# old-dab/rtlsdr

Hardware: NVIDIA B200
Metric: input Msamples/s (higher is better)
Workload: dtype int16/int64 fixed point

## Files before the change

### rtlsdr_b200/csrc/scan_abi.cu

```cuda
#include "../../include/rtlsdr_gpu_scan.h"
#include "csv_text.cuh"
#include "scan_kernels.cuh"
#include "scan_large.cuh"

#include <algorithm>
#include <cmath>
#include <cstdio>
#include <cstdlib>
#include <cstring>
#include <new>
#include <string>
#include <vector>

using namespace rscan;

namespace {

constexpr int kDescSlots = 4;
constexpr size_t kDefaultRing = 32u << 20;
constexpr size_t kScratchBudget = 512ull << 20;
constexpr int kChainMaxPasses = 7;
constexpr int kChainCap0 = 8192;
constexpr int kDecimChunks = 4;
constexpr size_t kDecimOverlapBytes = 1ull << 30;

enum Path { PATH_RMS, PATH_SMALL_U8, PATH_SMALL_DECIM, PATH_LARGE };

struct DescSlot {
	void *h = nullptr;
	void *d = nullptr;
	size_t cap = 0;
	cudaEvent_t done = nullptr;
	bool used = false;
};

struct RegularKey {
	const void *base = nullptr;
	int hop_first = -1, hop_count = 0, passes = 0;
	long long pass_stride = 0, hop_stride = 0;
	bool valid = false;
	int n_reads = 0, n_segs = 0;
	bool operator==(const RegularKey &o) const
	{
		return valid && o.valid && base == o.base && hop_first == o.hop_first && hop_count == o.hop_count &&
		       passes == o.passes && pass_stride == o.pass_stride && hop_stride == o.hop_stride;
	}
};

}

struct rtlsdr_gpu_scan {
	rtlsdr_gpu_scan_cfg_t cfg;
	int N = 1;
	Path path = PATH_SMALL_U8;
	int l_len = 0, n_blocks = 0, blocks_padded = 0, samples_per_read = 0;
	long long image_stride = 0;
	int db_i1 = 0, db_i2 = 0, db_count = 2;
	int num_sms = 148, ctas_per_sm = 2;

	cudaStream_t own_stream = nullptr, stream = nullptr;
	cudaEvent_t ev_a = nullptr, ev_b = nullptr;

	long long *d_avg = nullptr;
	long long *d_smp64 = nullptr;
	long long *d_avg_other = nullptr;
	cudaStream_t report_stream = nullptr;
	cudaEvent_t ev_scan = nullptr, ev_report[2] = { nullptr, nullptr };
	bool report_pending[2] = { false, false };
	int cur_acc = 0;
	unsigned *d_done = nullptr;
	unsigned long long *d_level = nullptr;
	std::vector<uint64_t> level_bytes;
	int2 *d_tw = nullptr;
	int2 *d_twc = nullptr;
	int2 *d_twb = nullptr;
	uint16_t *d_win = nullptr;
	double *d_db = nullptr;
	double *d_iir = nullptr;
	int *d_samples = nullptr;
	int *h_samples_pinned = nullptr;
	std::vector<int> samples;
	PassTw tw0;
	std::vector<int2> tw_host;

	size_t ring_bytes = 0;
	int ring_reads = 0;
	uint8_t *h_ring[2] = { nullptr, nullptr };
	uint8_t *d_ring[2] = { nullptr, nullptr };
	cudaEvent_t ring_done[2] = { nullptr, nullptr };
	bool ring_busy[2] = { false, false };
	int cur_half = 0;
	std::vector<int> ring_hops;
	std::vector<uint8_t> hop_shadow;

	DescSlot desc[kDescSlots];
	int desc_next = 0;
	struct RegCache {
		RegularKey key;
		void *d_desc = nullptr;
		size_t cap = 0;
		std::vector<int4> segs;
		uint64_t stamp = 0;
	};
	std::vector<RegCache> reg_cache;
	uint64_t reg_stamp = 0;
	cudaStream_t aux[2] = { nullptr, nullptr };
	cudaEvent_t fork_ev = nullptr, join_ev[2] = { nullptr, nullptr };
	cudaStream_t hb_head_stream = nullptr;
	cudaEvent_t hb_fork = nullptr, hb_join = nullptr;
	cudaStream_t copy_stream = nullptr;
	cudaEvent_t bulk_free = nullptr;
	bool bulk_used = false;
	std::vector<cudaEvent_t> chunk_ready;

	uint8_t *d_scratch = nullptr;
	size_t scratch_bytes = 0;

	uint8_t *d_bulk = nullptr;
	size_t bulk_bytes = 0;

	int2 *d_csv_cols = nullptr;
	int csv_rows = 0;
	double csv_step = 0.0;
	char *d_csv_slots = nullptr;
	size_t csv_slot_bytes = 0;
	int *d_csv_lens = nullptr;
	char *d_csv_text = nullptr;
	size_t csv_text_bytes = 0;
	long long *d_csv_len = nullptr;
	long long *h_csv_len = nullptr;

	bool last_was_epilogue = false;
	bool samples_on_device = false;
	uint64_t launches = 0, h2d = 0, d2h = 0;
	std::vector<std::pair<cudaEvent_t, cudaEvent_t>> timed;
	std::vector<cudaEvent_t> ev_pool;
	bool timing = false;
	int timing_every = 1;
	uint64_t timing_count = 0;

	int dbg_boxcar_mode = -1;
	int dbg_stagger_ns = 0;
	bool dbg_no_fused_boxcar = false, dbg_no_hb_stream = false, dbg_rms_warp = false;
	int dbg_large_pipe = 1;

	std::string last_error;
};

namespace {

#define CU(call)                                                                                 \
	do {                                                                                         \
		cudaError_t _e = (call);                                                                 \
		if (_e != cudaSuccess) {                                                                 \
			h->last_error = std::string(#call) + ": " + cudaGetErrorString(_e);                  \
			return RTLSDR_GPU_ERR_CUDA;                                                          \
		}                                                                                        \
	} while (0)

// ... 172 lines not shown
		return 0;
	}
	std::vector<int> count(tc + 1, 0);
	for (int i = 0; i < n; i++)
		count[hops[i] + 1]++;
	for (int i = 0; i < tc; i++)
		count[i + 1] += count[i];
	s_offs.resize(n);
	s_hops.resize(n);
	std::vector<int> cursor(count.begin(), count.end() - 1);
	for (int i = 0; i < n; i++) {
		int p = cursor[hops[i]]++;
		s_offs[p] = offs[i];
		s_hops[p] = hops[i];
	}
	segs.clear();
	if (h->path == PATH_SMALL_U8 || h->path == PATH_RMS || h->path == PATH_LARGE)
		return 0;
	const bool big_decim = h->path == PATH_SMALL_DECIM && (size_t)n * (size_t)h->cfg.buf_len >= kDecimOverlapBytes;
	const int target = std::max(1, h->num_sms * h->ctas_per_sm) * (big_decim ? kDecimChunks : 1);
	int chunk = std::max(1, (n + target - 1) / target);
	{
		const double per_seg = 0.35;
		double best = 1e300;
		int best_chunk = chunk;
		for (int k = 1; k <= 16; k++) {
			const int c = std::max(1, (chunk + k - 1) / k);
			long long nseg = 0;
			for (int hp = 0; hp < tc; hp++) {
				const int cnt = count[hp + 1] - count[hp];
				nseg += (cnt + c - 1) / c;
			}
			const long long rounds = (nseg + target - 1) / target;
			const double cost = (double)rounds * (c + per_seg);
			if (cost < best * 0.98) {
				best = cost;
				best_chunk = c;
			}
			if (c == 1)
				break;
		}
		chunk = best_chunk;
	}
	for (int hp = 0; hp < tc; hp++) {
		int lo = count[hp], hi = count[hp + 1];
		int cnt = hi - lo;
		if (cnt <= 0)
			continue;
		int pieces = (cnt + chunk - 1) / chunk;
		for (int k = 0; k < pieces; k++) {
			int a = lo + (int)((long long)cnt * k / pieces), b = lo + (int)((long long)cnt * (k + 1) / pieces);
			if (b > a)
				segs.push_back(make_int4(hp, a, b - a, 0));
		}
	}
	return (int)segs.size();
}


int large_process(rtlsdr_gpu_scan *h, const uint8_t *base, const long long *d_offs, const int *d_hops, int n_reads);

template <class K, class P>
int launch_after_epilogue(rtlsdr_gpu_scan *h, K kern, int grid, int block, int smem, const P &prm, bool allow_pdl = true)
{
	if (allow_pdl && h->last_was_epilogue && h->stream == h->own_stream) {
		cudaLaunchConfig_t cfg = {};
		cfg.gridDim = dim3(grid);
		cfg.blockDim = dim3(block);
		cfg.dynamicSmemBytes = smem;
		cfg.stream = h->stream;
		cudaLaunchAttribute attr[1];
		attr[0].id = cudaLaunchAttributeProgrammaticStreamSerialization;
		attr[0].val.programmaticStreamSerializationAllowed = 1;
		cfg.attrs = attr;
		cfg.numAttrs = 1;
		CU(cudaLaunchKernelEx(&cfg, kern, prm));
	} else {
		kern<<<grid, block, smem, h->stream>>>(prm);
	}
	h->last_was_epilogue = false;
	return 0;
}

template <int L, bool PEAK, bool IN16>
int launch_small_t(rtlsdr_gpu_scan *h, const SmallParams &prm)
{
	auto kern = scan_small_kernel<L, PEAK, IN16>;
	const int smem = SmallSmem<L>::bytes;
	static bool attr_set[64] = { false };
	if (h->cfg.device >= 64 || !attr_set[h->cfg.device]) {
		CU(cudaFuncSetAttribute(kern, cudaFuncAttributeMaxDynamicSharedMemorySize, smem));
		if (h->cfg.device < 64)
			attr_set[h->cfg.device] = true;
	}
	const int grid = IN16 ? std::min(prm.n_segs, h->num_sms * 8)
			      : (int)std::min<long long>(2ll * prm.n_entries, (long long)h->num_sms * h->ctas_per_sm);
	if (int rc = launch_after_epilogue(h, kern, grid, kThreads, smem, prm, !IN16))
		return rc;
	return check_launch(h, "scan_small_kernel");
}

template <int L>
int launch_small_l(rtlsdr_gpu_scan *h, const SmallParams &prm, bool in16)
{
	if (h->cfg.peak_hold)
		return in16 ? launch_small_t<L, true, true>(h, prm) : launch_small_t<L, true, false>(h, prm);
	return in16 ? launch_small_t<L, false, true>(h, prm) : launch_small_t<L, false, false>(h, prm);
}

int launch_small(rtlsdr_gpu_scan *h, const SmallParams &prm, bool in16)
{
	switch (h->cfg.bin_e) {
	case 1: return launch_small_l<1>(h, prm, in16);
	case 2: return launch_small_l<2>(h, prm, in16);
	case 3: return launch_small_l<3>(h, prm, in16);
	case 4: return launch_small_l<4>(h, prm, in16);
	case 5: return launch_small_l<5>(h, prm, in16);
	case 6: return launch_small_l<6>(h, prm, in16);
	case 7: return launch_small_l<7>(h, prm, in16);
	case 8: return launch_small_l<8>(h, prm, in16);
	case 9: return launch_small_l<9>(h, prm, in16);
	case 10: return launch_small_l<10>(h, prm, in16);
	case 11: return launch_small_l<11>(h, prm, in16);
	case 12: return launch_small_l<12>(h, prm, in16);
	default: break;
	}
	return RTLSDR_GPU_ERR_CONFIG;
}

template <int L, bool PEAK, int NS>
int launch_fused_boxcar_t(rtlsdr_gpu_scan *h, const FusedBoxcarParams &prm)
{
	auto k = scan_boxcar_fused_kernel<L, PEAK, NS>;
	const int smem = FusedSmem<L>::bytes(prm.ds, NS);
	const int grid = std::min(prm.n_segs, h->num_sms * 8);
	CU(cudaFuncSetAttribute(k, cudaFuncAttributeMaxDynamicSharedMemorySize, smem));
	if (int rc = launch_after_epilogue(h, k, grid, kThreads, smem, prm))
		return rc;
	return check_launch(h, "scan_boxcar_fused_kernel");
}

template <int L>
int launch_fused_boxcar_l(rtlsdr_gpu_scan *h, const FusedBoxcarParams &prm_in)
{
	FusedBoxcarParams prm = prm_in;
	const int limit = 227 * 1024 - 1024;
	int slots;
	if (2 * (FusedSmem<L>::bytes(prm.ds, 4) + 1024) <= 227 * 1024) {
		slots = 4;
	} else if (2 * (FusedSmem<L>::bytes(prm.ds, 3) + 1024) <= 227 * 1024) {
		slots = 3;
	} else {
		const int fit = (limit - FusedSmem<L>::off_stage) / (512 * prm.ds);
		slots = fit >= 12 ? 12 : fit >= 8 ? 8 : fit >= 6 ? 6 : fit >= 4 ? 4 : fit >= 3 ? 3 : 2;
	}
	prm.slots = slots;
	const bool pk = h->cfg.peak_hold != 0;
#define FUSED_CASE(NSV)                                                                               \
	case NSV:                                                                                     \
		return pk ? launch_fused_boxcar_t<L, true, NSV>(h, prm) : launch_fused_boxcar_t<L, false, NSV>(h, prm)
	switch (slots) {
		FUSED_CASE(12);
		FUSED_CASE(8);
		FUSED_CASE(6);
		FUSED_CASE(4);
		FUSED_CASE(3);
	default:
		return pk ? launch_fused_boxcar_t<L, true, 2>(h, prm) : launch_fused_boxcar_t<L, false, 2>(h, prm);
	}
#undef FUSED_CASE
}

constexpr int kStreamMinDs = 2;
constexpr int kStreamOneFftGroupDs = 24;

template <int L, int FG>
int stream_boxcar_slots(int ds)
{
	const int fit = (227 * 1024 - StreamSmem<L, FG>::off_stage) / (512 * ds);
	return std::min(fit, kStreamMaxSlots);
}

template <int L, bool PEAK, int FG, int BG>
int launch_stream_boxcar_t(rtlsdr_gpu_scan *h, const FusedBoxcarParams &prm_in)
{
	FusedBoxcarParams prm = prm_in;
	prm.slots = stream_boxcar_slots<L, FG>(prm.ds);
// ... 884 lines not shown
		delete h;
		return RTLSDR_GPU_ERR_CONFIG;
	}
	h->db_count = h->db_i2 - h->db_i1 + 2;

	int rc = RTLSDR_GPU_ERR_CUDA;
	do {
		if (cudaStreamCreateWithFlags(&h->own_stream, cudaStreamNonBlocking) != cudaSuccess)
			break;
		h->stream = h->own_stream;
		const size_t avg_bytes = ((size_t)cfg->tune_count * N + (size_t)cfg->tune_count) * sizeof(long long);
		if (cudaMalloc(&h->d_avg, avg_bytes) != cudaSuccess ||
		    cudaMalloc(&h->d_db, (size_t)cfg->tune_count * h->db_count * sizeof(double)) != cudaSuccess ||
		    cudaMalloc(&h->d_samples, (size_t)cfg->tune_count * sizeof(int)) != cudaSuccess ||
		    cudaMallocHost(&h->h_samples_pinned, (size_t)cfg->tune_count * sizeof(int)) != cudaSuccess) {
			rc = RTLSDR_GPU_ERR_NOMEM;
			break;
		}
		h->d_smp64 = h->d_avg + (size_t)cfg->tune_count * N;
		if (cfg->flags & RTLSDR_GPU_FLAG_ASYNC_REPORT) {
			if (cudaMalloc(&h->d_avg_other, avg_bytes) != cudaSuccess) {
				rc = RTLSDR_GPU_ERR_NOMEM;
				break;
			}
			if (cudaMemsetAsync(h->d_avg_other, 0, avg_bytes, h->stream) != cudaSuccess ||
			    cudaStreamCreateWithFlags(&h->report_stream, cudaStreamNonBlocking) != cudaSuccess ||
			    cudaEventCreateWithFlags(&h->ev_scan, cudaEventDisableTiming) != cudaSuccess ||
			    cudaEventCreateWithFlags(&h->ev_report[0], cudaEventDisableTiming) != cudaSuccess ||
			    cudaEventCreateWithFlags(&h->ev_report[1], cudaEventDisableTiming) != cudaSuccess)
				break;
		}
		if (cudaMalloc(&h->d_done, (size_t)cfg->tune_count * sizeof(unsigned)) != cudaSuccess) {
			rc = RTLSDR_GPU_ERR_NOMEM;
			break;
		}
		if (cudaMemsetAsync(h->d_done, 0, (size_t)cfg->tune_count * sizeof(unsigned), h->stream) != cudaSuccess)
			break;
		if (cudaMemsetAsync(h->d_avg, 0, avg_bytes, h->stream) != cudaSuccess)
			break;
		if (cfg->iir_alpha > 0.0) {
			const size_t ib = (size_t)cfg->tune_count * (size_t)(h->db_count - 1) * sizeof(double);
			if (cudaMalloc(&h->d_iir, ib) != cudaSuccess) {
				rc = RTLSDR_GPU_ERR_NOMEM;
				break;
			}
			if (cudaMemsetAsync(h->d_iir, 0xFF, ib, h->stream) != cudaSuccess)
				break;
		}
		if (cfg->flags & RTLSDR_GPU_FLAG_LEVEL_STATS) {
			const size_t lb = (size_t)cfg->tune_count * 2 * sizeof(unsigned long long);
			if (cudaMalloc(&h->d_level, lb) != cudaSuccess) {
				rc = RTLSDR_GPU_ERR_NOMEM;
				break;
			}
			if (cudaMemsetAsync(h->d_level, 0, lb, h->stream) != cudaSuccess)
				break;
			h->level_bytes.assign(cfg->tune_count, 0);
		}

		if (cfg->bin_e > 0) {
			std::vector<int16_t> sine((size_t)N * 3 / 4 + 4, 0);
			if (cfg->sinewave)
				memcpy(sine.data(), cfg->sinewave, ((size_t)N * 3 / 4) * sizeof(int16_t));
			else
				host_sine_table(cfg->bin_e, sine.data());
			const int half = std::max(N / 2, 1);
			h->tw_host.resize(half);
			for (int j = 0; j < half; j++) {
				int16_t wr = (int16_t)(sine[j + N / 4] >> 1);
				int16_t wi = (int16_t)((int16_t)(-sine[j]) >> 1);
				h->tw_host[j] = make_int2(wr, wi);
			}
			if (h->tw_host[0].y != 0 || (N >= 4 && h->tw_host[N / 4].x != 0)) {
				rc = RTLSDR_GPU_ERR_CONFIG;
				break;
			}
			memset(&h->tw0, 0, sizeof(h->tw0));
			for (int b = 0; b < 4 && b < cfg->bin_e; b++)
				for (int g = 0; g < (1 << b); g++)
					h->tw0.w[(1 << b) - 1 + g] = h->tw_host[(size_t)g << (cfg->bin_e - 1 - b)];
			std::vector<uint16_t> win(N);
			for (int i = 0; i < N; i++)
				win[i] = (uint16_t)((cfg->window_coefs ? cfg->window_coefs[i] : 256) & 0xFFFF);
			if (cudaMalloc(&h->d_tw, (size_t)half * sizeof(int2)) != cudaSuccess ||
			    cudaMalloc(&h->d_win, (size_t)N * sizeof(uint16_t)) != cudaSuccess) {
				rc = RTLSDR_GPU_ERR_NOMEM;
				break;
			}
			if (cudaMemcpy(h->d_tw, h->tw_host.data(), (size_t)half * sizeof(int2), cudaMemcpyHostToDevice) != cudaSuccess ||
			    cudaMemcpy(h->d_win, win.data(), (size_t)N * sizeof(uint16_t), cudaMemcpyHostToDevice) != cudaSuccess)
				break;
		}

		if (cfg->bin_e > 4 && cfg->bin_e <= 12) {
			const int L = cfg->bin_e;
			std::vector<int2> twc((size_t)N - 16);
			for (int st = 4; st < L; st++)
				for (int m = 0; m < (1 << st); m++)
					twc[(size_t)(1 << st) - 16 + m] = h->tw_host[(size_t)m << (L - 1 - st)];
			if (cudaMalloc(&h->d_twc, twc.size() * sizeof(int2)) != cudaSuccess) {
				rc = RTLSDR_GPU_ERR_NOMEM;
				break;
			}
			if (cudaMemcpy(h->d_twc, twc.data(), twc.size() * sizeof(int2), cudaMemcpyHostToDevice) != cudaSuccess)
				break;
		}
		if (h->path == PATH_LARGE) {
			std::vector<int2> twc(240);
			for (int st = 4; st < 8; st++)
				for (int m = 0; m < (1 << st); m++)
					twc[(size_t)(1 << st) - 16 + m] = h->tw_host[(size_t)m << (cfg->bin_e - 1 - st)];
			if (cudaMalloc(&h->d_twc, twc.size() * sizeof(int2)) != cudaSuccess) {
				rc = RTLSDR_GPU_ERR_NOMEM;
				break;
			}
			if (cudaMemcpy(h->d_twc, twc.data(), twc.size() * sizeof(int2), cudaMemcpyHostToDevice) != cudaSuccess)
				break;
		}
		if (h->path == PATH_LARGE) {
			const int L = cfg->bin_e, lb = std::min(8, L - 8);
			std::vector<int2> twb((size_t)256 * 240, make_int2(0, 0));
			for (int se = 4; se < lb; se++)
				for (int plow = 0; plow < 256; plow++)
					for (int ilow = 0; ilow < (1 << se); ilow++)
						twb[(size_t)256 * ((1 << se) - 16) + ((size_t)plow << se) + ilow] =
							h->tw_host[((size_t)((ilow << 8) | plow)) << (L - 9 - se)];
			if (cudaMalloc(&h->d_twb, twb.size() * sizeof(int2)) != cudaSuccess) {
				rc = RTLSDR_GPU_ERR_NOMEM;
				break;
			}
			if (cudaMemcpy(h->d_twb, twb.data(), twb.size() * sizeof(int2), cudaMemcpyHostToDevice) != cudaSuccess)
				break;
		}

		size_t ring = cfg->ring_bytes ? cfg->ring_bytes : kDefaultRing;
		const size_t B = (size_t)cfg->buf_len;
		h->ring_reads = (int)std::max<size_t>(1, ring / B);
		h->ring_bytes = (size_t)h->ring_reads * B;
		bool ok = true;
		for (int i = 0; i < 2 && ok; i++) {
			ok = cudaMallocHost(&h->h_ring[i], h->ring_bytes) == cudaSuccess &&
			     cudaMalloc(&h->d_ring[i], h->ring_bytes) == cudaSuccess &&
			     cudaEventCreateWithFlags(&h->ring_done[i], cudaEventDisableTiming) == cudaSuccess;
		}
		if (!ok) {
			rc = RTLSDR_GPU_ERR_NOMEM;
			break;
		}
		h->ring_hops.reserve(h->ring_reads);
		if (cfg->flags & RTLSDR_GPU_FLAG_SHORT_READS)
			h->hop_shadow.assign((size_t)cfg->tune_count * B, 0);
		if (cudaStreamSynchronize(h->stream) != cudaSuccess)
			break;
		rc = 0;
	} while (0);
	if (rc) {
		cudaGetLastError();
		free_all(h);
		return rc;
	}
	*out = h;
	return 0;
}

void rtlsdr_gpu_scan_close(rtlsdr_gpu_scan_t *h)
{
// ... 680 lines not shown
```

### rtlsdr_b200/csrc/scan_compat.cuh

```cuda
#pragma once
#include <stdint.h>

#ifdef SCAN_EMU
#include "cuda_emu.h"
#define SCAN_DYN_SMEM(name) unsigned char *name = ::cuda_emu::dyn_smem()
#define SCAN_GRID_CONSTANT
#else
#include <cuda_runtime.h>
#define SCAN_DYN_SMEM(name) extern __shared__ __align__(16) unsigned char name[]
#define SCAN_GRID_CONSTANT __grid_constant__
#endif

#define SCAN_DEV __device__ __forceinline__

namespace rscan {

SCAN_DEV void cp_async16(void *smem_dst, const void *gmem_src)
{
#ifdef SCAN_EMU
	::cuda_emu::copy16(smem_dst, gmem_src);
#else
	unsigned s = (unsigned)__cvta_generic_to_shared(smem_dst);
	asm volatile("cp.async.cg.shared.global [%0], [%1], 16;\n" ::"r"(s), "l"(gmem_src) : "memory");
#endif
}

SCAN_DEV void cp_async8(void *smem_dst, const void *gmem_src)
{
#ifdef SCAN_EMU
	::cuda_emu::copy8(smem_dst, gmem_src);
#else
	unsigned s = (unsigned)__cvta_generic_to_shared(smem_dst);
	asm volatile("cp.async.ca.shared.global [%0], [%1], 8;\n" ::"r"(s), "l"(gmem_src) : "memory");
#endif
}

SCAN_DEV void cp_async_commit()
{
#ifndef SCAN_EMU
	asm volatile("cp.async.commit_group;\n" ::: "memory");
#endif
}

SCAN_DEV void cp_async_wait_all()
{
#ifndef SCAN_EMU
	asm volatile("cp.async.wait_group 0;\n" ::: "memory");
#endif
}

SCAN_DEV void cp_async_wait_pending(int pending)
{
#ifndef SCAN_EMU
	switch (pending) {
	case 0: asm volatile("cp.async.wait_group 0;\n" ::: "memory"); break;
	case 1: asm volatile("cp.async.wait_group 1;\n" ::: "memory"); break;
	case 2: asm volatile("cp.async.wait_group 2;\n" ::: "memory"); break;
	default: asm volatile("cp.async.wait_group 3;\n" ::: "memory"); break;
	}
#else
	(void)pending;
#endif
}

template <int PENDING>
SCAN_DEV void cp_async_wait_group()
{
#ifndef SCAN_EMU
	asm volatile("cp.async.wait_group %0;\n" ::"n"(PENDING) : "memory");
#endif
}

SCAN_DEV void pdl_wait()
{
#ifndef SCAN_EMU
	asm volatile("griddepcontrol.wait;\n" ::: "memory");
#endif
}

SCAN_DEV void pdl_launch_dependents()
{
#ifndef SCAN_EMU
	asm volatile("griddepcontrol.launch_dependents;\n" ::: "memory");
#endif
}

SCAN_DEV void mbar_init(uint64_t *bar, int count)
{
#ifdef SCAN_EMU
	::cuda_emu::mbar_init(bar, count);
#else
	unsigned s = (unsigned)__cvta_generic_to_shared(bar);
	asm volatile("mbarrier.init.shared::cta.b64 [%0], %1;\n" ::"r"(s), "r"(count) : "memory");
#endif
}

SCAN_DEV void mbar_fence_init()
{
#ifndef SCAN_EMU
	asm volatile("fence.mbarrier_init.release.cluster;\n" ::: "memory");
	asm volatile("fence.proxy.async.shared::cta;\n" ::: "memory");
#endif
}

SCAN_DEV void mbar_arrive(uint64_t *bar)
{
#ifdef SCAN_EMU
	::cuda_emu::mbar_arrive(bar, 0);
#else
	unsigned s = (unsigned)__cvta_generic_to_shared(bar);
	asm volatile("{\n.reg .b64 st;\nmbarrier.arrive.shared::cta.b64 st, [%0];\n}\n" ::"r"(s) : "memory");
#endif
}

SCAN_DEV void mbar_arrive_expect_tx(uint64_t *bar, unsigned bytes)
{
#ifdef SCAN_EMU
	::cuda_emu::mbar_arrive(bar, bytes);
#elif defined(RSCAN_RACECHECK_COPY)
	(void)bar; (void)bytes;
#else
	unsigned s = (unsigned)__cvta_generic_to_shared(bar);
	asm volatile("{\n.reg .b64 st;\nmbarrier.arrive.expect_tx.shared::cta.b64 st, [%0], %1;\n}\n" ::"r"(s), "r"(bytes)
		     : "memory");
#endif
}

SCAN_DEV void mbar_wait(uint64_t *bar, unsigned parity)
{
#ifdef SCAN_EMU
	::cuda_emu::mbar_wait(bar, parity);
#else
	unsigned s = (unsigned)__cvta_generic_to_shared(bar);
	asm volatile("{\n"
		     ".reg .pred p;\n"
		     "MBAR_WAIT:\n"
		     "mbarrier.try_wait.parity.shared::cta.b64 p, [%0], %1;\n"
		     "@p bra MBAR_DONE;\n"
		     "bra MBAR_WAIT;\n"
		     "MBAR_DONE:\n"
		     "}\n" ::"r"(s),
		     "r"(parity)
		     : "memory");
#endif
}

SCAN_DEV void bulk_copy_g2s(void *smem_dst, const void *gmem_src, unsigned bytes, uint64_t *bar)
{
#ifdef SCAN_EMU
	::cuda_emu::bulk_copy(smem_dst, gmem_src, bytes, bar);
#elif defined(RSCAN_RACECHECK_COPY)
	{
		const uint4 *s = (const uint4 *)gmem_src;
		uint4 *d = (uint4 *)smem_dst;
		for (unsigned i = 0; i < bytes / 16; ++i)
			d[i] = s[i];
		__threadfence_block();
		mbar_arrive(bar);
	}
#else
	unsigned d = (unsigned)__cvta_generic_to_shared(smem_dst);
	unsigned b = (unsigned)__cvta_generic_to_shared(bar);
	asm volatile("cp.async.bulk.shared::cluster.global.mbarrier::complete_tx::bytes [%0], [%1], %2, [%3];\n" ::"r"(d),
		     "l"(gmem_src), "r"(bytes), "r"(b)
		     : "memory");
#endif
// ... 22 lines not shown
```

### rtlsdr_b200/csrc/scan_kernels.cuh

```cuda
#pragma once
#include "scan_compat.cuh"

#ifndef RSCAN_WIN_REGS
#define RSCAN_WIN_REGS 1
#endif
#ifndef RSCAN_FRONT_IDP
#define RSCAN_FRONT_IDP 1
#endif
#ifndef RSCAN_PACKED_B
#define RSCAN_PACKED_B 1
#endif

namespace rscan {

typedef uint32_t c16;

constexpr int kThreads = 256;
constexpr int kPts     = 16;
constexpr int kWS      = kThreads * kPts;
constexpr int kStageBytes = 16384;
constexpr int kXchWords   = kWS + kWS / 16;


SCAN_DEV int c16_re(c16 v) { return (int)(int16_t)(uint16_t)(v & 0xFFFFu); }
SCAN_DEV int c16_im(c16 v) { return ((int32_t)v) >> 16; }
SCAN_DEV c16 c16_pack(int re, int im) { return ((uint32_t)re & 0xFFFFu) | ((uint32_t)im << 16); }

SCAN_DEV int fix_mpy(int w, int x) { return (w * x + 16384) >> 15; }

SCAN_DEV void butterfly(c16 &a, c16 &b, int wr, int wi)
{
	const int br = c16_re(b), bi = c16_im(b);
	const int tr = fix_mpy(wr, br) - fix_mpy(wi, bi);
	const int ti = fix_mpy(wr, bi) + fix_mpy(wi, br);
	const int qr = c16_re(a) >> 1, qi = c16_im(a) >> 1;
	b = c16_pack(qr - tr, qi - ti);
	a = c16_pack(qr + tr, qi + ti);
}

struct X2 {
	int re, im;
};

SCAN_DEV X2 x_unpack(c16 v)
{
	X2 x;
	x.re = (int)(v << 16);
	x.im = (int)v;
	return x;
}

SCAN_DEV c16 x_pack(X2 x)
{
	return __byte_perm((uint32_t)x.re, (uint32_t)x.im, 0x7632);
}

SCAN_DEV int c16_re_fast(c16 v)
{
#ifdef SCAN_EMU
	return (int)(int16_t)(uint16_t)(v & 0xFFFFu);
#else
	int r;
	asm("prmt.b32 %0, %1, 0, 0x9910;" : "=r"(r) : "r"(v));
	return r;
#endif
}

SCAN_DEV void butterfly_x(X2 &a, X2 &b, int wr, int wi);

SCAN_DEV void butterfly_x_packed_b(X2 &a, X2 &b, c16 vb, int wr, int wi)
{
	const int br = c16_re_fast(vb), bi = ((int)vb) >> 16;
	const int tr = ((wr * br + 16384) >> 15) - ((wi * bi + 16384) >> 15);
	const int ti = ((wr * bi + 16384) >> 15) + ((wi * br + 16384) >> 15);
	const int hr = a.re >> 1, hi = a.im >> 1;
	b.re = hr - tr * 65536;
	b.im = hi - ti * 65536;
	a.re = hr + tr * 65536;
	a.im = hi + ti * 65536;
}

SCAN_DEV void butterfly_x(X2 &a, X2 &b, int wr, int wi)
{
	const int br = b.re >> 16, bi = b.im >> 16;
	const int tr = ((wr * br + 16384) >> 15) - ((wi * bi + 16384) >> 15);
	const int ti = ((wr * bi + 16384) >> 15) + ((wi * br + 16384) >> 15);
	const int hr = a.re >> 1, hi = a.im >> 1;
	b.re = hr - tr * 65536;
	b.im = hi - ti * 65536;
	a.re = hr + tr * 65536;
	a.im = hi + ti * 65536;
}

SCAN_DEV void butterfly_x_re(X2 &a, X2 &b, int wr)
{
	const int tr = (wr * (b.re >> 16) + 16384) >> 15;
	const int ti = (wr * (b.im >> 16) + 16384) >> 15;
	const int hr = a.re >> 1, hi = a.im >> 1;
	b.re = hr - tr * 65536;
	b.im = hi - ti * 65536;
	a.re = hr + tr * 65536;
	a.im = hi + ti * 65536;
}

SCAN_DEV void butterfly_x_im(X2 &a, X2 &b, int wi)
{
	const int tr = -((wi * (b.im >> 16) + 16384) >> 15);
	const int ti = (wi * (b.re >> 16) + 16384) >> 15;
	const int hr = a.re >> 1, hi = a.im >> 1;
	b.re = hr - tr * 65536;
	b.im = hi - ti * 65536;
	a.re = hr + tr * 65536;
	a.im = hi + ti * 65536;
}

template <bool PEAK>
SCAN_DEV void accumulate_power(unsigned long long &acc, int re, int im)
{
	const unsigned pw = (unsigned)(re * re) + (unsigned)(im * im);
	if constexpr (PEAK)
		acc = acc > pw ? acc : (unsigned long long)pw;
	else
		acc += pw;
}


template <int K>
SCAN_DEV int pos(int t, int r)
{
	constexpr int sh = 4 * K;
	return ((t >> sh) << (sh + 4)) | (r << sh) | (t & ((1 << sh) - 1));
}

SCAN_DEV int xch_idx(int p) { return p + (p >> 4); }

SCAN_DEV constexpr int brev4(int r)
{
	return ((r & 1) << 3) | ((r & 2) << 1) | ((r & 4) >> 1) | ((r & 8) >> 3);
}

SCAN_DEV int brev_bits(unsigned v, int bits)
{
	return bits <= 0 ? 0 : (int)(__brev(v) >> (32 - bits));
}

template <int K, int LE, class TW>
SCAN_DEV void run_pass(X2 (&x)[kPts], int t, const TW &tw, const c16 *packed = nullptr)
{
	constexpr int s0 = 4 * K;
	constexpr int ns = (LE - s0) < 4 ? (LE - s0) : 4;
#pragma unroll
	for (int b = 0; b < ns; ++b) {
#pragma unroll
		for (int r = 0; r < kPts; ++r) {
			if ((r & (1 << b)) == 0) {
				const int2 w = tw.template get<K>(s0 + b, pos<K>(t, r));
				const int g = r & ((1 << b) - 1);
				if (RSCAN_PACKED_B && K > 0 && b == 0 && packed)
					butterfly_x_packed_b(x[r], x[r | 1], packed[r | 1], w.x, w.y);
				else if (K == 0 && TW::kTrivial && g == 0)
					butterfly_x_re(x[r], x[r | (1 << b)], w.x);
				else if (K == 0 && TW::kTrivial && b > 0 && g == (1 << (b - 1)))
					butterfly_x_im(x[r], x[r | (1 << b)], w.y);
				else
					butterfly_x(x[r], x[r | (1 << b)], w.x, w.y);
			}
		}
	}
}

struct BlockBar {
	SCAN_DEV void sync() const { __syncthreads(); }
};
struct GroupBar {
	int id, count;
	SCAN_DEV void sync() const { named_bar_sync(id, count); }
};

template <int KA, int KB, bool LEAD, class BAR = BlockBar>
SCAN_DEV void exchange(X2 (&x)[kPts], c16 *xch, int tw_, int t, const BAR &bar = BAR())
{
	if (LEAD)
		bar.sync();
#pragma unroll
	for (int r = 0; r < kPts; ++r)
		xch[xch_idx(pos<KA>(tw_, r))] = x_pack(x[r]);
	bar.sync();
#pragma unroll
	for (int r = 0; r < kPts; ++r)
		x[r] = x_unpack(xch[xch_idx(pos<KB>(t, r))]);
}

template <int KA, int KB, class BAR>
SCAN_DEV void exchange_pk(X2 (&x)[kPts], c16 (&pk)[kPts], c16 *xch, int tw_, int t, const BAR &bar)
{
#pragma unroll
	for (int r = 0; r < kPts; ++r)
		xch[xch_idx(pos<KA>(tw_, r))] = x_pack(x[r]);
	bar.sync();
#pragma unroll
	for (int r = 0; r < kPts; ++r) {
		pk[r] = xch[xch_idx(pos<KB>(t, r))];
		if (!RSCAN_PACKED_B || (r & 1) == 0)
			x[r] = x_unpack(pk[r]);
	}
}

template <int L>
SCAN_DEV int front_thread_map(int t, int &t0)
{
	if constexpr (L == 12) {
		const int b = brev_bits((unsigned)(t & 31), 5), w = t >> 5;
		const int g = (b << 3) | ((((b >> 3) & 3) ^ (w & 3)) << 1) | (w >> 2);
		t0 = brev_bits((unsigned)g, 8);
		return g;
	} else {
		t0 = t;
		if constexpr (L >= 4)
			return brev_bits((unsigned)(t & ((1 << (L - 4)) - 1)), L - 4);
		return 0;
	}
}

template <int LE, class TW>
SCAN_DEV void engine_fft(X2 (&x)[kPts], c16 *xch, int t, const TW &tw)
{
	run_pass<0, LE>(x, t, tw);
	if constexpr (LE > 4) {
		exchange<0, 1, true>(x, xch, t, t);
		run_pass<1, LE>(x, t, tw);
	}
	if constexpr (LE > 8) {
		exchange<1, 2, true>(x, xch, t, t);
		run_pass<2, LE>(x, t, tw);
	}
}

template <int LE, class TW, class BAR = BlockBar>
SCAN_DEV void engine_fft_db(X2 (&x)[kPts], c16 *xch2, int &flip, int t, const TW &tw, const BAR &bar = BAR(), int t0 = -1)
{
	if (t0 < 0)
		t0 = t;
	run_pass<0, LE>(x, t0, tw);
	c16 pk[kPts];
	if constexpr (LE > 4) {
		exchange_pk<0, 1, BAR>(x, pk, xch2 + flip * kXchWords, t0, t, bar);
		flip ^= 1;
		run_pass<1, LE>(x, t, tw, pk);
	}
	if constexpr (LE > 8) {
		exchange_pk<1, 2, BAR>(x, pk, xch2 + flip * kXchWords, t, t, bar);
		flip ^= 1;
		run_pass<2, LE>(x, t, tw, pk);
	}
}

template <int LE>
SCAN_DEV int last_pos(int t, int r)
{
	return pos<(LE - 1) / 4>(t, r);
}


struct PassTw {
	int2 w[15];
};

struct SmallParams {
	const uint8_t *base;
	const long long *read_off;
	long long regular_stride;
	int entry_base;
	const int4 *segs;
	int n_segs;
	const int *hop_of;
	int n_entries;
	int stagger_ns;
	long long *avg;
	long long *samples;
	int samples_per_read;
	const int2 *tw;
	const int2 *twc;
	const uint16_t *win;
	const int *dc_ave;
	int l_len;
	int n_blocks;
	int blocks_padded;
	PassTw tw0;
};

template <int L>
struct SmallSmem {
	static constexpr int N = 1 << L;
	static constexpr int off_stage = 0;
	static constexpr int off_xch = 2 * kStageBytes;
	static constexpr int off_tw = off_xch + 2 * kXchWords * 4;
	static constexpr int tw_entries = N > 16 ? N - 16 : 1;
	static constexpr int off_win = (off_tw + tw_entries * 8 + 15) & ~15;
	static constexpr int off_red = (off_win + N * 2 + 15) & ~15;
	static constexpr int off_dck = off_red + 16 * 8;
	static constexpr int bytes = off_dck + 16;
};

template <int L>
struct TwSmall {
	static constexpr bool kTrivial = true;
	const int2 *tws;
	const PassTw *tw0;
	template <int K>
	SCAN_DEV int2 get(int s, int pa) const
	{
		const int m = pa & ((1 << s) - 1);
		if constexpr (K == 0)
			return tw0->w[(1 << s) - 1 + m];
		else
			return tws[(1 << s) - 16 + m];
	}
};

template <int L>
SCAN_DEV void load_tables(int2 *tws, uint16_t *wins, const int2 *twc, const uint16_t *win, int t, int stride)
{
	constexpr int N = 1 << L;
	if constexpr (N > 16) {
		for (int i = t; i < (N - 16) / 2; i += stride)
			cp_async16((uint8_t *)tws + 16 * i, (const uint8_t *)twc + 16 * i);
	}
	if constexpr (N >= 8) {
		for (int i = t; i < N / 8; i += stride)
			cp_async16((uint8_t *)wins + 16 * i, (const uint8_t *)win + 16 * i);
	} else {
		for (int i = t; i < N; i += stride)
			wins[i] = win[i];
	}
}

SCAN_DEV long long entry_offset(const SmallParams &prm, int e)
{
	return prm.read_off ? prm.read_off[e] : (long long)(e - prm.entry_base) * prm.regular_stride;
}

SCAN_DEV int dc_average(long long sum, int length)
{
	return (int)(int16_t)(sum / (long long)length);
}


SCAN_DEV void u8_read_dc(const uint8_t *st, int *red, int t, int &kI, int &kQ)
{
	unsigned sI = 0, sQ = 0;
#pragma unroll
	for (int i = 0; i < kStageBytes / (kThreads * 16); ++i) {
		const uint4 q = *(const uint4 *)(st + (i * kThreads + t) * 16);
		sI = __dp4a(q.x, 0x00010001u, sI);
		sQ = __dp4a(q.x, 0x01000100u, sQ);
		sI = __dp4a(q.y, 0x00010001u, sI);
		sQ = __dp4a(q.y, 0x01000100u, sQ);
		sI = __dp4a(q.z, 0x00010001u, sI);
		sQ = __dp4a(q.z, 0x01000100u, sQ);
		sI = __dp4a(q.w, 0x00010001u, sI);
		sQ = __dp4a(q.w, 0x01000100u, sQ);
	}
#pragma unroll
	for (int o = 16; o > 0; o >>= 1) {
		sI += __shfl_xor_sync(0xffffffffu, sI, o);
		sQ += __shfl_xor_sync(0xffffffffu, sQ, o);
	}
	if ((t & 31) == 0) {
		red[(t >> 5) * 2 + 0] = (int)sI;
		red[(t >> 5) * 2 + 1] = (int)sQ;
	}
	__syncthreads();
	int tI = 0, tQ = 0;
#pragma unroll
	for (int w = 0; w < kThreads / 32; ++w) {
		tI += red[w * 2];
		tQ += red[w * 2 + 1];
	}
	kI = 127 + (int)(int16_t)((tI - 127 * (kStageBytes / 2)) / kStageBytes);
	kQ = 127 + (int)(int16_t)((tQ - 127 * (kStageBytes / 2)) / (kStageBytes - 1));
}

template <int L>
SCAN_DEV void front_index(int r, int t, int trev, int blkbase, int &nblk, int &n)
{
	constexpr int N = 1 << L;
	if constexpr (L >= 4) {
		nblk = (brev4(r) << (L - 4)) + trev;
		n = blkbase + nblk;
	} else {
		nblk = brev_bits((unsigned)(r & (N - 1)), L);
		n = (t << 4) + (r & ~(N - 1)) + nblk;
	}
}


constexpr int kWinRegs = kPts / 2;

template <int L>
SCAN_DEV void load_window_regs(unsigned (&wreg)[kWinRegs], const uint16_t *wins, int t, int trev, int blkbase)
{
#pragma unroll
	for (int j = 0; j < kWinRegs; ++j) {
		int nblk0, nblk1, n;
		front_index<L>(2 * j, t, trev, blkbase, nblk0, n);
		front_index<L>(2 * j + 1, t, trev, blkbase, nblk1, n);
		wreg[j] = (unsigned)wins[nblk0] | ((unsigned)wins[nblk1] << 16);
	}
}

template <int L, bool WREG = false>
SCAN_DEV void front_u8(X2 (&x)[kPts], const uint8_t *st, int ws, int kI, int kQ, const uint16_t *wins, int t, int trev,
		       int blkbase, const unsigned *wreg = nullptr)
{
#pragma unroll
	for (int r = 0; r < kPts; ++r) {
		int nblk, n;
		front_index<L>(r, t, trev, blkbase, nblk, n);
		unsigned wx;
		if constexpr (WREG)
			wx = (r & 1) ? (wreg[r >> 1] & 0xFFFF0000u) : (wreg[r >> 1] << 16);
		else
			wx = (unsigned)wins[nblk] << 16;
		const unsigned raw = ((const uint16_t *)st)[ws * kWS + n];
#if RSCAN_FRONT_IDP
		x[r].re = (int)(__dp4a(raw, 0x00000001u, (unsigned)-kI) * wx);
		x[r].im = (int)(__dp4a(raw, 0x00000100u, (unsigned)-kQ) * wx);
#else
		x[r].re = (int)((unsigned)((int)(raw & 0xFFu) - kI) * wx);
		x[r].im = (int)((unsigned)((int)(raw >> 8) - kQ) * wx);
#endif
	}
}

template <int L, bool PEAK, class BAR = BlockBar>
SCAN_DEV void flush_bins(unsigned long long (&acc)[kPts], long long *out, unsigned long long *bins, int t,
			 const BAR &bar = BAR())
{
	constexpr int N = 1 << L;
	if constexpr (L == 12) {
#pragma unroll
		for (int r = 0; r < kPts; ++r) {
			const int bin = last_pos<L>(t, r) & (N - 1);
			if constexpr (PEAK)
				atomicMax(out + bin, (long long)acc[r]);
			else
				atomicAdd((unsigned long long *)(out + bin), acc[r]);
		}
	} else {
		bar.sync();
		for (int i = t; i < N; i += kThreads)
			bins[i] = 0ull;
		bar.sync();
#pragma unroll
		for (int r = 0; r < kPts; ++r) {
			const int bin = last_pos<L>(t, r) & (N - 1);
			if constexpr (PEAK)
				atomicMax(bins + bin, acc[r]);
			else
				atomicAdd(bins + bin, acc[r]);
		}
		bar.sync();
		for (int i = t; i < N; i += kThreads) {
			if constexpr (PEAK)
				atomicMax(out + i, (long long)bins[i]);
			else
				atomicAdd((unsigned long long *)(out + i), bins[i]);
		}
		bar.sync();
	}
}

template <int L, bool PEAK, bool IN16>
__global__ void __launch_bounds__(kThreads, 2)
scan_small_kernel(const SCAN_GRID_CONSTANT SmallParams prm)
{
	SCAN_DYN_SMEM(smem);
	typedef SmallSmem<L> SM;
	constexpr int N = 1 << L;
	uint8_t *stage = smem + SM::off_stage;
	c16 *xch = (c16 *)(smem + SM::off_xch);
	int2 *tws = (int2 *)(smem + SM::off_tw);
	uint16_t *wins = (uint16_t *)(smem + SM::off_win);
	int *red = (int *)(smem + SM::off_red);

	const int t = threadIdx.x;
	load_tables<L>(tws, wins, prm.twc, prm.win, t, kThreads);

	TwSmall<L> tw;
	tw.tws = tws;
	tw.tw0 = &prm.tw0;

	int blkbase = 0, t0;
	const int trev = front_thread_map<L>(t, t0);
	if constexpr (L >= 4)
		blkbase = (t >> (L - 4)) << L;

	int flip = 0;

	if constexpr (!IN16) {
		const long long total_ws = 2ll * prm.n_entries;
		long long ws_lo, ws_hi;
		if (total_ws >= 8ll * gridDim.x) {
			ws_lo = total_ws * blockIdx.x / gridDim.x;
			ws_hi = total_ws * (blockIdx.x + 1) / gridDim.x;
		} else {
			ws_lo = 2 * ((long long)prm.n_entries * blockIdx.x / gridDim.x);
			ws_hi = 2 * ((long long)prm.n_entries * (blockIdx.x + 1) / gridDim.x);
		}
		if (ws_lo >= ws_hi)
			return;
#ifndef SCAN_EMU
		if (prm.stagger_ns > 0 && blockIdx.x >= gridDim.x / 2)
			__nanosleep((unsigned)prm.stagger_ns);
#endif
		const int e_lo = (int)(ws_lo >> 1), e_hi = (int)((ws_hi + 1) >> 1);

		unsigned long long acc[kPts];
#pragma unroll
		for (int r = 0; r < kPts; ++r)
			acc[r] = 0ull;
		int hop = prm.hop_of[e_lo], hop_ws = 0;
		bool waited = false;

		{
			const uint8_t *src = prm.base + prm.read_off[e_lo];
#pragma unroll
			for (int i = 0; i < kStageBytes / (kThreads * 16); ++i)
				cp_async16(stage + (i * kThreads + t) * 16, src + (i * kThreads + t) * 16);
			cp_async_commit();
		}
		constexpr bool kWinRegsOn = RSCAN_WIN_REGS && L == 12;
		unsigned wreg[kWinRegs];
		if constexpr (kWinRegsOn) {
			cp_async_wait_all();
			__syncthreads();
			load_window_regs<L>(wreg, wins, t, trev, blkbase);
		}
		for (int e = e_lo; e < e_hi; ++e) {
			const int u = e - e_lo;
			cp_async_wait_all();
			__syncthreads();
			int next_hop = -1;
			if (e + 1 < e_hi) {
				const uint8_t *src = prm.base + prm.read_off[e + 1];
				uint8_t *dst = stage + ((u + 1) & 1) * kStageBytes;
#pragma unroll
				for (int i = 0; i < kStageBytes / (kThreads * 16); ++i)
					cp_async16(dst + (i * kThreads + t) * 16, src + (i * kThreads + t) * 16);
				cp_async_commit();
				next_hop = prm.hop_of[e + 1];
			}
			const uint8_t *st = stage + (u & 1) * kStageBytes;
			int kI, kQ;
			u8_read_dc(st, red, t, kI, kQ);

			const int ws0 = (2ll * e < ws_lo) ? 1 : 0, ws1 = (2ll * e + 2 > ws_hi) ? 1 : 2;
#pragma unroll 1
			for (int ws = ws0; ws < ws1; ++ws) {
				X2 x[kPts];
				front_u8<L, kWinRegsOn>(x, st, ws, kI, kQ, wins, t, trev, blkbase, wreg);
				engine_fft_db<L>(x, xch, flip, t, tw, BlockBar(), t0);
#pragma unroll
				for (int r = 0; r < kPts; ++r)
					accumulate_power<PEAK>(acc[r], x[r].re >> 16, x[r].im >> 16);
			}
			hop_ws += ws1 - ws0;

			if (next_hop != hop) {
				if (!waited)
					pdl_wait();
				waited = true;
				if (t == 0)
					atomicAdd((unsigned long long *)(prm.samples + hop),
						  (unsigned long long)((long long)hop_ws * (prm.samples_per_read / 2)));
				flush_bins<L, PEAK>(acc, prm.avg + ((long long)hop << L), (unsigned long long *)xch, t);
#pragma unroll
				for (int r = 0; r < kPts; ++r)
					acc[r] = 0ull;
				hop = next_hop;
				hop_ws = 0;
			}
		}
	} else {
	for (int seg = blockIdx.x; seg < prm.n_segs; seg += gridDim.x) {
		const int4 sg = prm.segs[seg];
		const int hop = sg.x, first = sg.y;
		const int seg_blocks = sg.z * prm.blocks_padded;
		const int units = (int)(((long long)seg_blocks * N + kWS - 1) / kWS);

		unsigned long long acc[kPts];
#pragma unroll
		for (int r = 0; r < kPts; ++r)
			acc[r] = 0ull;

		{
			const uint8_t *src = prm.base + entry_offset(prm, first);
#pragma unroll
			for (int i = 0; i < kStageBytes / (kThreads * 16); ++i)
				cp_async16(stage + (i * kThreads + t) * 16, src + (i * kThreads + t) * 16);
			cp_async_commit();
		}

		for (int u = 0; u < units; ++u) {
			cp_async_wait_all();
			__syncthreads();
			if (u + 1 < units) {
				const uint8_t *src = prm.base + entry_offset(prm, first) + (long long)(u + 1) * kStageBytes;
				uint8_t *dst = stage + ((u + 1) & 1) * kStageBytes;
#pragma unroll
				for (int i = 0; i < kStageBytes / (kThreads * 16); ++i)
					cp_async16(dst + (i * kThreads + t) * 16, src + (i * kThreads + t) * 16);
				cp_async_commit();
			}
			const uint8_t *st = stage + (u & 1) * kStageBytes;

			int limI = kWS, limQ = kWS, kI, kQ;
			if constexpr (L >= 4) {
				const int gb = u * (kWS / N) + (t >> (L - 4));
				const int rd = gb / prm.blocks_padded, bir = gb - rd * prm.blocks_padded;
				const bool live = gb < seg_blocks && bir < prm.n_blocks;
				const int e = first + (live ? rd : 0) - prm.entry_base;
				kI = __ldg(prm.dc_ave + 2 * e);
				kQ = __ldg(prm.dc_ave + 2 * e + 1);
				limI = live ? ((prm.l_len + 1) >> 1) - bir * N : 0;
				limQ = live ? (prm.l_len >> 1) - bir * N : 0;
			} else {
				kI = kQ = 0;
			}

			X2 x[kPts];
#pragma unroll
			for (int r = 0; r < kPts; ++r) {
				int nblk, n;
				front_index<L>(r, t, trev, blkbase, nblk, n);
				const int wv = wins[nblk];
				const c16 raw = ((const c16 *)st)[n];
				int re = c16_re(raw), im = c16_im(raw);
				if constexpr (L >= 4) {
					if (nblk < limI)
						re -= kI;
					if (nblk < limQ)
						im -= kQ;
				} else {
					const int gb = u * (kWS / N) + (n >> L);
// ... 1731 lines not shown
```

Before: 266,000.

## Add unit-window u8 front end, int2 exchange FFT for 4096 bins, faster DC reduce

Detects at setup when every window coefficient equals 256 and dispatches a specialized 4096-bin u8 kernel. That kernel skips the per-sample window multiply and builds the shifted sample with a single mad. The 4096-point path also gets a new exchange routine that stores full int2 values in shared memory with explicit barriers, replacing the double-buffered exchange, and the DC-estimate reduction now uses __reduce_add_sync with vectorized shared reads. The unit-window path only runs for the default or flat window, and the new exchange adds a barrier per window step.

```diff
diff --git a/rtlsdr_b200/csrc/scan_abi.cu b/rtlsdr_b200/csrc/scan_abi.cu
--- a/rtlsdr_b200/csrc/scan_abi.cu
+++ b/rtlsdr_b200/csrc/scan_abi.cu
@@ -75,6 +75,7 @@
 	int2 *d_twc = nullptr;
 	int2 *d_twb = nullptr;
 	uint16_t *d_win = nullptr;
+	bool win_unit = false;
 	double *d_db = nullptr;
 	double *d_iir = nullptr;
 	int *d_samples = nullptr;
@@ -413,10 +414,10 @@
 	return 0;
 }
 
-template <int L, bool PEAK, bool IN16>
+template <int L, bool PEAK, bool IN16, bool UNITW = false>
 int launch_small_t(rtlsdr_gpu_scan *h, const SmallParams &prm)
 {
-	auto kern = scan_small_kernel<L, PEAK, IN16>;
+	auto kern = scan_small_kernel<L, PEAK, IN16, UNITW>;
 	const int smem = SmallSmem<L>::bytes;
 	static bool attr_set[64] = { false };
 	if (h->cfg.device >= 64 || !attr_set[h->cfg.device]) {
@@ -434,6 +435,10 @@
 template <int L>
 int launch_small_l(rtlsdr_gpu_scan *h, const SmallParams &prm, bool in16)
 {
+	if constexpr (L == 12) {
+		if (!in16 && h->win_unit)
+			return h->cfg.peak_hold ? launch_small_t<L, true, false, true>(h, prm) : launch_small_t<L, false, false, true>(h, prm);
+	}
 	if (h->cfg.peak_hold)
 		return in16 ? launch_small_t<L, true, true>(h, prm) : launch_small_t<L, true, false>(h, prm);
 	return in16 ? launch_small_t<L, false, true>(h, prm) : launch_small_t<L, false, false>(h, prm);
@@ -1484,6 +1489,7 @@
 			std::vector<uint16_t> win(N);
 			for (int i = 0; i < N; i++)
 				win[i] = (uint16_t)((cfg->window_coefs ? cfg->window_coefs[i] : 256) & 0xFFFF);
+			h->win_unit = window_is_unit(win.data(), N);
 			if (cudaMalloc(&h->d_tw, (size_t)half * sizeof(int2)) != cudaSuccess ||
 			    cudaMalloc(&h->d_win, (size_t)N * sizeof(uint16_t)) != cudaSuccess) {
 				rc = RTLSDR_GPU_ERR_NOMEM;
diff --git a/rtlsdr_b200/csrc/scan_compat.cuh b/rtlsdr_b200/csrc/scan_compat.cuh
--- a/rtlsdr_b200/csrc/scan_compat.cuh
+++ b/rtlsdr_b200/csrc/scan_compat.cuh
@@ -82,6 +82,17 @@
 {
 #ifndef SCAN_EMU
 	asm volatile("griddepcontrol.launch_dependents;\n" ::: "memory");
+#endif
+}
+
+SCAN_DEV unsigned warp_sum(unsigned v)
+{
+#ifdef SCAN_EMU
+	for (int o = 16; o > 0; o >>= 1)
+		v += __shfl_xor_sync(0xffffffffu, v, o);
+	return v;
+#else
+	return __reduce_add_sync(0xffffffffu, v);
 #endif
 }
 
diff --git a/rtlsdr_b200/csrc/scan_kernels.cuh b/rtlsdr_b200/csrc/scan_kernels.cuh
--- a/rtlsdr_b200/csrc/scan_kernels.cuh
+++ b/rtlsdr_b200/csrc/scan_kernels.cuh
@@ -62,6 +62,17 @@
 #else
 	int r;
 	asm("prmt.b32 %0, %1, 0, 0x9910;" : "=r"(r) : "r"(v));
+	return r;
+#endif
+}
+
+SCAN_DEV unsigned imad_u32(unsigned a, unsigned b, unsigned c)
+{
+#ifdef SCAN_EMU
+	return a * b + c;
+#else
+	unsigned r;
+	asm("mad.lo.u32 %0, %1, %2, %3;" : "=r"(r) : "r"(a), "r"(b), "r"(c));
 	return r;
 #endif
 }
@@ -206,6 +217,23 @@
 	}
 }
 
+template <int KA, int KB>
+SCAN_DEV void exchange_x8(X2 (&x)[kPts], int2 *xch, bool lead, int tw_, int t)
+{
+	if (lead)
+		__syncthreads();
+#pragma unroll
+	for (int r = 0; r < kPts; ++r)
+		xch[xch_idx(pos<KA>(tw_, r))] = make_int2(x[r].re, x[r].im);
+	__syncthreads();
+#pragma unroll
+	for (int r = 0; r < kPts; ++r) {
+		const int2 v = xch[xch_idx(pos<KB>(t, r))];
+		x[r].re = v.x;
+		x[r].im = v.y;
+	}
+}
+
 template <int L>
 SCAN_DEV int front_thread_map(int t, int &t0)
 {
@@ -253,6 +281,16 @@
 		flip ^= 1;
 		run_pass<2, LE>(x, t, tw, pk);
 	}
+}
+
+template <class TW>
+SCAN_DEV void engine_fft_x8(X2 (&x)[kPts], int2 *xch, bool lead, int t, int t0, const TW &tw)
+{
+	run_pass<0, 12>(x, t0, tw);
+	exchange_x8<0, 1>(x, xch, lead, t0, t);
+	run_pass<1, 12>(x, t, tw);
+	exchange_x8<1, 2>(x, xch, true, t, t);
+	run_pass<2, 12>(x, t, tw);
 }
 
 template <int LE>
@@ -361,21 +399,17 @@
 		sI = __dp4a(q.w, 0x00010001u, sI);
 		sQ = __dp4a(q.w, 0x01000100u, sQ);
 	}
-#pragma unroll
-	for (int o = 16; o > 0; o >>= 1) {
-		sI += __shfl_xor_sync(0xffffffffu, sI, o);
-		sQ += __shfl_xor_sync(0xffffffffu, sQ, o);
-	}
-	if ((t & 31) == 0) {
-		red[(t >> 5) * 2 + 0] = (int)sI;
-		red[(t >> 5) * 2 + 1] = (int)sQ;
-	}
+	sI = warp_sum(sI);
+	sQ = warp_sum(sQ);
+	if ((t & 31) == 0)
+		*(int2 *)(red + (t >> 5) * 2) = make_int2((int)sI, (int)sQ);
 	__syncthreads();
 	int tI = 0, tQ = 0;
 #pragma unroll
-	for (int w = 0; w < kThreads / 32; ++w) {
-		tI += red[w * 2];
-		tQ += red[w * 2 + 1];
+	for (int w = 0; w < kThreads / 32; w += 2) {
+		const int4 v = *(const int4 *)(red + w * 2);
+		tI += v.x + v.z;
+		tQ += v.y + v.w;
 	}
 	kI = 127 + (int)(int16_t)((tI - 127 * (kStageBytes / 2)) / kStageBytes);
 	kQ = 127 + (int)(int16_t)((tQ - 127 * (kStageBytes / 2)) / (kStageBytes - 1));
@@ -409,7 +443,17 @@
 	}
 }
 
-template <int L, bool WREG = false>
+inline bool window_is_unit(const uint16_t *win, int n)
+{
+	for (int i = 0; i < n; i++)
+		if (win[i] != 256)
+			return false;
+	return true;
+}
+
+enum WinSrc { kWinShared, kWinInRegs, kWinUnit };
+
+template <int L, int WIN = kWinShared>
 SCAN_DEV void front_u8(X2 (&x)[kPts], const uint8_t *st, int ws, int kI, int kQ, const uint16_t *wins, int t, int trev,
 		       int blkbase, const unsigned *wreg = nullptr)
 {
@@ -417,12 +461,17 @@
 	for (int r = 0; r < kPts; ++r) {
 		int nblk, n;
 		front_index<L>(r, t, trev, blkbase, nblk, n);
+		const unsigned raw = ((const uint16_t *)st)[ws * kWS + n];
+		if constexpr (WIN == kWinUnit) {
+			x[r].re = (int)imad_u32(raw, 1u << 24, (unsigned)-kI << 24);
+			x[r].im = (int)(__dp4a(raw, 0x00000100u, (unsigned)-kQ) << 24);
+			continue;
+		}
 		unsigned wx;
-		if constexpr (WREG)
+		if constexpr (WIN == kWinInRegs)
 			wx = (r & 1) ? (wreg[r >> 1] & 0xFFFF0000u) : (wreg[r >> 1] << 16);
 		else
 			wx = (unsigned)wins[nblk] << 16;
-		const unsigned raw = ((const uint16_t *)st)[ws * kWS + n];
 #if RSCAN_FRONT_IDP
 		x[r].re = (int)(__dp4a(raw, 0x00000001u, (unsigned)-kI) * wx);
 		x[r].im = (int)(__dp4a(raw, 0x00000100u, (unsigned)-kQ) * wx);
@@ -471,10 +520,11 @@
 	}
 }
 
-template <int L, bool PEAK, bool IN16>
+template <int L, bool PEAK, bool IN16, bool UNITW = false>
 __global__ void __launch_bounds__(kThreads, 2)
 scan_small_kernel(const SCAN_GRID_CONSTANT SmallParams prm)
 {
+	static_assert(!UNITW || (L == 12 && !IN16), "the unit-window front end is the 4096-bin u8 one");
 	SCAN_DYN_SMEM(smem);
 	typedef SmallSmem<L> SM;
 	constexpr int N = 1 << L;
@@ -530,9 +580,9 @@
 				cp_async16(stage + (i * kThreads + t) * 16, src + (i * kThreads + t) * 16);
 			cp_async_commit();
 		}
-		constexpr bool kWinRegsOn = RSCAN_WIN_REGS && L == 12;
+		constexpr int kWin = UNITW ? kWinUnit : (RSCAN_WIN_REGS && L == 12) ? kWinInRegs : kWinShared;
 		unsigned wreg[kWinRegs];
-		if constexpr (kWinRegsOn) {
+		if constexpr (kWin == kWinInRegs) {
 			cp_async_wait_all();
 			__syncthreads();
 			load_window_regs<L>(wreg, wins, t, trev, blkbase);
@@ -559,8 +609,11 @@
 #pragma unroll 1
 			for (int ws = ws0; ws < ws1; ++ws) {
 				X2 x[kPts];
-				front_u8<L, kWinRegsOn>(x, st, ws, kI, kQ, wins, t, trev, blkbase, wreg);
-				engine_fft_db<L>(x, xch, flip, t, tw, BlockBar(), t0);
+				front_u8<L, kWin>(x, st, ws, kI, kQ, wins, t, trev, blkbase, wreg);
+				if constexpr (L == 12)
+					engine_fft_x8(x, (int2 *)xch, ws != ws0, t, t0, tw);
+				else
+					engine_fft_db<L>(x, xch, flip, t, tw, BlockBar(), t0);
 #pragma unroll
 				for (int r = 0; r < kPts; ++r)
 					accumulate_power<PEAK>(acc[r], x[r].re >> 16, x[r].im >> 16);
```

Result: faster. 273,100 (median of 6 runs) (+2.7%).
